# JJKK1313/DiTreeOnlinePlanner

Hardware: AMD Instinct MI355X
Metric: candidate tree-expansions/sec (carmaze, H=32) (higher is better)
Workload: dtype f16x3; 1 GPU; cfgs/carmaze.yaml + fm_policy flow sampler (K=1), batch=1024 candidates per GPU, H=32 (4 chunks x 8 steps), boxes.csv 20x20, 1024-node tree snapshot, seeded random weights; batch_per_gpu=1024, global_batch=1024, edge_length=32, action_horizon=8, pred_horizon=64, flow_steps=1, tree_nodes=1024, parallelism=candidates sharded x1

## Files before the change

### ditreeonlineplanner_amd/csrc/conv_tiles.hip

```cpp
#include <type_traits>

#include "denoise_device.h"

static thread_local bool g_dn_dry_run = false;
void denoise_set_dry_run(bool on) { g_dn_dry_run = on; }
bool denoise_dry_run() { return g_dn_dry_run; }

template <int PREC>
__device__ __forceinline__ void gemm_epilogue(const ConvGemmParams& p, f32x16_t (&acc)[2][4], char* smem, int tm, int tn,
                                              int tid, int lane, int r5, int h, int wm, int wn,
                                              long long out_extra_bytes = 0) {

  constexpr int ET = PREC == 2 ? 1 : 0;
  float satm = 0.0f;
  const int c_l = wn * 128 + 4 * r5;
  const int n0 = tn * 256 + c_l;
  const bool n_ok = n0 < p.N;
  float bias4[4] = {0.f, 0.f, 0.f, 0.f};
  if (p.bias != nullptr && n_ok) {
    f32x4_t t = *(const f32x4_t*)(p.bias + n0);
#pragma unroll
    for (int j = 0; j < 4; ++j) bias4[j] = t[j];
  }
#pragma unroll
// ... 1115 lines not shown
    __builtin_amdgcn_sched_group_barrier(0x008, 16, 0);
    __builtin_amdgcn_sched_barrier(0);
    PSTAMP(3);
    mm16(1, 0, 0);
    if constexpr (ISSUE_A && T != 2) {
      if constexpr (T == 0) { issue_a(v + 1, 0); issue_a(v + 1, 1); issue_a(v + 1, 2); }
      else { issue_a(v + 1, 3); issue_a(v + 1, 4); if constexpr (NP == 6) issue_a(v + 1, 5); }
      __builtin_amdgcn_sched_group_barrier(0x008, 4, 2);
      __builtin_amdgcn_sched_group_barrier(0x020, 1, 2);
      __builtin_amdgcn_sched_group_barrier(0x008, 4, 2);
      __builtin_amdgcn_sched_group_barrier(0x020, 1, 2);
      __builtin_amdgcn_sched_group_barrier(0x008, 4, 2);
      if constexpr (T == 0 || NP == 6) __builtin_amdgcn_sched_group_barrier(0x020, 1, 2);
      __builtin_amdgcn_sched_group_barrier(0x008, 4, 2);
    }
    __builtin_amdgcn_sched_barrier(0);
    PSTAMP(4);
    __builtin_amdgcn_s_setprio(0);
    mm16(0, 1, 1);
    __builtin_amdgcn_sched_barrier(0);
    PSTAMP(5);
    if constexpr (HAS_NEXT) {
      if constexpr (VM == 0) asm volatile("s_waitcnt vmcnt(0) lgkmcnt(0)" ::: "memory");
      else if constexpr (VM == 3) asm volatile("s_waitcnt vmcnt(3) lgkmcnt(0)" ::: "memory");
      else asm volatile("s_waitcnt vmcnt(2) lgkmcnt(0)" ::: "memory");
      __builtin_amdgcn_s_barrier();
      __builtin_amdgcn_s_setprio(3);
      PSTAMP(6);
      constexpr int T1 = (T + 1) % 3;
      rdA(0, v + (T + 1) / 3, T1, 0);
      rdB(0, v + (T + 1) / 3, T1, 1, 0);
    }
    constexpr int T2 = (T + 2) % 3;
    const int v2 = v + (T + 2) / 3;
#pragma unroll
    for (int mb = 0; mb < 4; ++mb)
#pragma unroll
      for (int jj = 0; jj < 4; ++jj) {
        mm(1, 1, 1, mb, (mb & 1) ? 3 - jj : jj);
        const int i = mb * 4 + jj;
        const int d = (i & 1) ? -1 : (i >> 1);
        if constexpr (ISSUE_W) { if (d >= 0 && d < 4) issue_w(v2, T2, d); }
      }
    if constexpr (HAS_NEXT) __builtin_amdgcn_sched_group_barrier(0x100, 8, 1);
    constexpr int NV = ISSUE_W ? 4 : 0;
#pragma unroll
    for (int i = 0; i < 16; ++i) {
      __builtin_amdgcn_sched_group_barrier(0x008, 1, 1);
      if (!(i & 1) && (i >> 1) < NV) __builtin_amdgcn_sched_group_barrier(0x020, 1, 1);
    }
    __builtin_amdgcn_sched_barrier(0);
    PSTAMP(7);
  };
#undef PSTAMP
  using I0 = std::integral_constant<int, 0>;
  using I1 = std::integral_constant<int, 1>;
  using I2 = std::integral_constant<int, 2>;
  using I3 = std::integral_constant<int, 3>;
  using Tt = std::true_type;
  using Ff = std::false_type;

#ifdef HALO16_STAMP
  const unsigned long long xs0 = __builtin_amdgcn_s_memrealtime();
#endif
#pragma unroll
  for (int i = 0; i < NP; ++i) issue_a(v_lo, i);
#pragma unroll
  for (int q = 0; q < 4; ++q) issue_w(v_lo, 0, q);
  asm volatile("s_waitcnt vmcnt(0)" ::: "memory");
  __builtin_amdgcn_s_barrier();
#pragma unroll
  for (int q = 0; q < 4; ++q) issue_w(v_lo, 1, q);
  rdA(0, v_lo, 0, 0);
  rdB(0, v_lo, 0, 1, 0);
#ifdef HALO16_STAMP
  const unsigned long long xs1 = __builtin_amdgcn_s_memrealtime();
#endif

  using IT1 = std::integral_constant<int, NP == 6 ? 3 : 2>;
  for (int v = v_lo; v < nv - 2; ++v) {
    step(I0{}, Tt{}, Tt{}, Tt{}, I3{}, v);
    step(I1{}, Tt{}, Tt{}, Tt{}, IT1{}, v);
    step(I2{}, Tt{}, Tt{}, Tt{}, I0{}, v);
  }
#ifdef X3_PHASE_STAMP
  if (blockIdx.x == 100 && lane == 0 && nv == 64) {
#pragma unroll
    for (int k = 0; k < 24; ++k) g_x3_phase[w][k] = pst[k];
    g_x3_phase[w][24] = (unsigned)nv;
  }
#endif
  {
    const int v = nv - 2;
    step(I0{}, Tt{}, Tt{}, Tt{}, I0{}, v);
    step(I1{}, Tt{}, Tt{}, Tt{}, I0{}, v);
    step(I2{}, Tt{}, Tt{}, Ff{}, I0{}, v);
  }
  {
    const int v = nv - 1;
    step(I0{}, Tt{}, Tt{}, Ff{}, I0{}, v);
    step(I1{}, Tt{}, Ff{}, Ff{}, I0{}, v);
    step(I2{}, Ff{}, Ff{}, Ff{}, I0{}, v);
  }
  __builtin_amdgcn_s_setprio(0);
  __syncthreads();
#ifdef HALO16_STAMP
  const unsigned long long xs2 = __builtin_amdgcn_s_memrealtime();
#endif
  if constexpr (SPLITK) {
    const int ntiles = ntm * ntn;
    float* mine = p.sk_ws + ((size_t)blockIdx.y * ntiles + tile) * 65536;
#pragma unroll
    for (int mb = 0; mb < 4; ++mb)
#pragma unroll
      for (int j = 0; j < 8; ++j) *(f32x4_t*)(mine + ((mb * 8 + j) * 512 + tid) * 4) = acc[mb][j];
    __threadfence();
    __syncthreads();
    int* s_last = (int*)smem;
    if (tid == 0) *s_last = atomicAdd(p.sk_cnt + tile, 1) == p.splitk - 1;
    __syncthreads();
    const bool last = *s_last != 0;
    __syncthreads();
    if (!last) return;
    __threadfence();
#pragma unroll
    for (int mb = 0; mb < 4; ++mb)
#pragma unroll
      for (int j = 0; j < 8; ++j) acc[mb][j] = f32x4_t{0.f, 0.f, 0.f, 0.f};
    for (int sp = 0; sp < p.splitk; ++sp) {
      const float* sl = p.sk_ws + ((size_t)sp * ntiles + tile) * 65536;
#pragma unroll
      for (int mb = 0; mb < 4; ++mb)
#pragma unroll
        for (int j = 0; j < 8; ++j) acc[mb][j] += *(const f32x4_t*)(sl + ((mb * 8 + j) * 512 + tid) * 4);
    }
    if (tid == 0) p.sk_cnt[tile] = 0;
  }
  gemm_epilogue16<ET, true, SHORT>(p, acc, smem, tm, tn, tid, lane, r4, h4, wm, wn);
#ifdef HALO16_STAMP
  __syncthreads();
  if (tid == 0) {
    const unsigned long long xs3 = __builtin_amdgcn_s_memrealtime();
    const unsigned int k = atomicAdd(&g_x3_count, 1u);
    if (k < X3_STAMP_MAX) {
      g_x3_stamp[k][0] = xs0; g_x3_stamp[k][1] = xs1; g_x3_stamp[k][2] = xs2; g_x3_stamp[k][3] = xs3;
      g_x3_stamp[k][4] = ((unsigned long long)nv << 32) | blockIdx.x;
      g_x3_stamp[k][5] = ((unsigned long long)__builtin_amdgcn_s_getreg((31 << 11) | 20) << 32) |
                         (unsigned int)__builtin_amdgcn_s_getreg((31 << 11) | 4);
    }
  }
#endif
}

template <int ET, bool SPLIT>
__global__ void __launch_bounds__(256) conv2d_small_kernel(ConvGemmParams p) {
  extern __shared__ __attribute__((aligned(16))) char smem[];
  constexpr int STAGE = 16384;
  constexpr int CK = SPLIT ? 32 : 64;
  const int tid = threadIdx.x, lane = tid & 63;
  const int w = __builtin_amdgcn_readfirstlane(tid >> 6);
  const int r5 = lane & 31, h = lane >> 5;
  const int wm = w >> 1, wn = w & 1;
  const int ntn = p.N >> 6;
  const int tm = blockIdx.x / ntn, tn = blockIdx.x - tm * ntn;
  const int kpt = p.Cin / CK;
  const long long K = (long long)p.taps * p.Cin;
  int k0 = 0, nk = p.taps * kpt;
  long long out_extra = 0;
  if (p.splitk > 1) {
    const int per = (nk + p.splitk - 1) / p.splitk;
    k0 = blockIdx.y * per;
    nk = min(nk - k0, per);
    out_extra = (long long)blockIdx.y * p.slab_stride;
  }

  const char* a_base[2];
  int ih0[2], iw0[2];
  const char* w_src[2];
  int slot_b[2];
  long long plane_a[2];
#pragma unroll
  for (int q = 0; q < 2; ++q) {
    const int r = (2 * w + q) * 8 + (lane >> 3);
    const int slot = (lane & 7) ^ ((r >> 1) & 7);
    slot_b[q] = SPLIT ? (slot & 3) * 16 : slot * 16;
    plane_a[q] = (SPLIT && (slot & 4)) ? p.a_plane : 0;
    const long long plane_w = (SPLIT && (slot & 4)) ? p.w_plane : 0;
    int m = tm * 64 + r;
    m = m < p.M ? m : p.M - 1;
    const int b = m / p.c2_OHW, rem = m - b * p.c2_OHW;
    const int oh = rem / p.c2_OW, ow = rem - oh * p.c2_OW;
    a_base[q] = (const char*)p.A + (long long)b * p.c2_H * p.c2_W * p.Cin * 2;
    ih0[q] = oh * p.c2_stride - p.c2_pad;
    iw0[q] = ow * p.c2_stride - p.c2_pad;
    w_src[q] = (const char*)p.W + ((long long)(tn * 64 + r) * K) * 2 + slot_b[q] + plane_w;
  }
  auto issue = [&](int kl) {
    const int k = k0 + kl;
    const int tap = k / kpt, kin = k - tap * kpt;
    const int kh = p.c2_kh[tap], kw = p.c2_kw[tap];
    char* st = smem + (kl % 3) * STAGE;
#pragma unroll
    for (int q = 0; q < 2; ++q) {
      const int ih = ih0[q] + kh, iw = iw0[q] + kw;
      const bool ok = ih >= 0 && ih < p.c2_H && iw >= 0 && iw < p.c2_W;
      const char* src = ok ? a_base[q] + ((long long)(ih * p.c2_W + iw) * p.Cin + kin * CK) * 2 + plane_a[q] : (const char*)p.zero;
      __builtin_amdgcn_global_load_lds((const GLOBAL_AS void*)(src + slot_b[q]), (LDS_AS void*)(st + (2 * w + q) * 1024), 16, 0, 0);
    }
#pragma unroll
    for (int q = 0; q < 2; ++q)
      __builtin_amdgcn_global_load_lds((const GLOBAL_AS void*)(w_src[q] + (long long)k * (CK * 2)),
                                       (LDS_AS void*)(st + 8192 + (2 * w + q) * 1024), 16, 0, 0);
  };

  f32x16_t acc;
#pragma unroll
  for (int i = 0; i < 16; ++i) acc[i] = 0.0f;
  const int a_row = wm * 32 + r5, b_row = wn * 32 + r5;
  const int a_off = a_row * 128, b_off = 8192 + b_row * 128;
  const int sa = (a_row >> 1) & 7, sb = (b_row >> 1) & 7;

  issue(0);
  if (nk > 1) issue(1);
  for (int k = 0; k < nk; ++k) {
    if (k + 1 < nk) asm volatile("s_waitcnt vmcnt(4)" ::: "memory");
    else asm volatile("s_waitcnt vmcnt(0)" ::: "memory");
    __builtin_amdgcn_s_barrier();
    if (k + 2 < nk) issue(k + 2);
    const char* st = smem + (k % 3) * STAGE;
    if constexpr (SPLIT) {
      short8_t af[4], bf[4];
#pragma unroll
      for (int ks = 0; ks < 4; ++ks) {
        af[ks] = *(const short8_t*)(st + a_off + ((((ks << 1) | h) ^ sa) << 4));
        bf[ks] = *(const short8_t*)(st + b_off + ((((ks << 1) | h) ^ sb) << 4));
      }
#pragma unroll
      for (int kk = 0; kk < 2; ++kk) acc = mfma32<ET>(af[kk], bf[kk + 2], acc);
#pragma unroll
      for (int kk = 0; kk < 2; ++kk) acc = mfma32<ET>(af[kk], bf[kk], acc);
#pragma unroll
      for (int kk = 0; kk < 2; ++kk) acc = mfma32<ET>(af[kk + 2], bf[kk], acc);
    } else {
#pragma unroll
      for (int ks = 0; ks < 4; ++ks) {
        const short8_t af = *(const short8_t*)(st + a_off + ((((ks << 1) | h) ^ sa) << 4));
        const short8_t bf = *(const short8_t*)(st + b_off + ((((ks << 1) | h) ^ sb) << 4));
        acc = mfma32<ET>(af, bf, acc);
      }
    }
    asm volatile("s_waitcnt lgkmcnt(0)" ::: "memory");
  }

  const int n = tn * 64 + wn * 32 + r5;
  float bias = (p.bias != nullptr && k0 == 0) ? p.bias[n] : 0.0f;
#pragma unroll
  for (int i = 0; i < 16; ++i) {
    const int m = tm * 64 + wm * 32 + (i & 3) + 8 * (i >> 2) + 4 * h;
    if (m < p.M) ((float*)p.Out)[out_extra + (long long)m * p.ldc + p.out_coff + n] = (ET == 1 ? acc[i] * p.w_scale : acc[i]) + bias;
  }
}

template <int ET, bool SPLIT, bool SHORT = false>
__global__ void __launch_bounds__(512, 2) gemm16_kernel(ConvGemmParams p) {
  extern __shared__ __attribute__((aligned(16))) char smem[];
  constexpr int BUF = 32768, W_BASE = 2 * BUF;
  const int tid = threadIdx.x, lane = tid & 63;
  const int w = __builtin_amdgcn_readfirstlane(tid >> 6);
  const int r4 = lane & 15, h4 = lane >> 4;
  const int wm = w >> 1, wn = w & 1;
  const int ntn = p.N >> 8, ntm = p.M >> 8;
  const int tile = xcd_remap_strips(blockIdx.x, ntm, ntn, p.xcd_strips);
  const int tm = tile / ntn, tn = tile - tm * ntn;
  constexpr int KB = SPLIT ? 64 : 128;
  const int nc = SPLIT ? (p.Cin >> 5) : (p.Cin >> 6), nk = p.taps * nc;
  const unsigned a_plane = (unsigned)p.a_plane, w_plane = (unsigned)p.w_plane;
  const long long K = (long long)p.taps * p.Cin;

  long long a_tile0;
  {
    const int m0 = tm * 256;
    const int b0 = m0 / p.L, l0 = m0 - b0 * p.L;
    a_tile0 = (((long long)b0 * p.in_Lp + (long long)l0 * p.in_stride + p.in_off) * p.lda) * 2;
  }
  const __amdgpu_buffer_rsrc_t a_rsrc =
      __builtin_amdgcn_make_buffer_rsrc((void*)((const char*)p.A + a_tile0), 0, 0x7fffffff, 0x00020000);
  const __amdgpu_buffer_rsrc_t w_rsrc =
      __builtin_amdgcn_make_buffer_rsrc((void*)((const char*)p.W + ((long long)tn * 256) * K * 2), 0, 0x7fffffff, 0x00020000);
  unsigned pae, pao, pbe, pbo;
  int aq[4], wq[4];
  {
    const int lr = lane >> 3;
    const int slot0 = (lane & 7) ^ (lr >> 1), slot1 = slot0 ^ 4;
    const int lrb = lr / p.L, lro = lrb * p.in_Lp + (lr - lrb * p.L) * p.in_stride;
    if constexpr (SPLIT) {
      pae = (unsigned)((lro * p.lda + (slot0 & 3) * 8) * 2) + ((slot0 & 4) ? a_plane : 0u);
      pao = (unsigned)((lro * p.lda + (slot1 & 3) * 8) * 2) + ((slot1 & 4) ? a_plane : 0u);
      pbe = (unsigned)(((long long)(8 * lr) * K + (slot0 & 3) * 8) * 2) + ((slot0 & 4) ? w_plane : 0u);
      pbo = (unsigned)(((long long)(8 * lr) * K + (slot1 & 3) * 8) * 2) + ((slot1 & 4) ? w_plane : 0u);
    } else {
      pae = (unsigned)((lro * p.lda + slot0 * 8) * 2);
      pao = (unsigned)((lro * p.lda + slot1 * 8) * 2);
      pbe = (unsigned)(((long long)(8 * lr) * K + slot0 * 8) * 2);
      pbo = (unsigned)(((long long)(8 * lr) * K + slot1 * 8) * 2);
    }
#pragma unroll
    for (int q = 0; q < 4; ++q) {
      const int r0 = (w * 4 + q) * 8;
      const int m = tm * 256 + r0;
      const int b = m / p.L, l = m - b * p.L;
      aq[q] = (int)((((long long)b * p.in_Lp + (long long)l * p.in_stride + p.in_off) * p.lda) * 2 - a_tile0);
      const int cu = (r0 & 128) + 8 * (r0 & 8) + ((r0 >> 4) & 7);
      wq[q] = (int)((long long)cu * K * 2);
    }
  }
  const int tap_bytes = p.lda * 2;
  auto src_off = [&](int k, int& ao, int& wo) {
    const int t = k / nc, c = k - t * nc;
    ao = t * tap_bytes + c * KB;
    wo = k * KB;
  };
  auto issue = [&](int kv) {
    int ao, wo;
    src_off(kv, ao, wo);
    char* ab = smem + (kv & 1) * BUF;
    char* wb = smem + W_BASE + (kv & 1) * BUF;
#pragma unroll
    for (int q = 0; q < 4; ++q)
      __builtin_amdgcn_raw_ptr_buffer_load_lds(a_rsrc, (LDS_AS void*)(ab + (w * 4 + q) * 1024), 16, (q & 1) ? pao : pae,
                                               aq[q] + ao, 0, 0);
#pragma unroll
    for (int q = 0; q < 4; ++q)
      __builtin_amdgcn_raw_ptr_buffer_load_lds(w_rsrc, (LDS_AS void*)(wb + (w * 4 + q) * 1024), 16, (q & 1) ? pbo : pbe,
                                               wq[q] + wo, 0, 0);
  };

  auto issue_wq = [&](int kv, int q) {
    int ao, wo;
    src_off(kv, ao, wo);
    __builtin_amdgcn_raw_ptr_buffer_load_lds(w_rsrc, (LDS_AS void*)(smem + W_BASE + (kv & 1) * BUF + (w * 4 + q) * 1024), 16,
                                             (q & 1) ? pbo : pbe, wq[q] + wo, 0, 0);
  };
  const int a_row = wm * 64 + r4;
  const int swa = (a_row >> 1) & 7;
  const int a_off = a_row * 128, b_off = (wn * 128 + r4) * 128;
  const int swb = (r4 >> 1) & 7;

  f32x4_t acc[4][8];
#pragma unroll
  for (int mb = 0; mb < 4; ++mb)
#pragma unroll
    for (int j = 0; j < 8; ++j) acc[mb][j] = f32x4_t{0.f, 0.f, 0.f, 0.f};
  short8_t af[2][4], bq[2][4];
  auto rdA = [&](int set, int k, int ks) {
    const char* ab = smem + (k & 1) * BUF + a_off + ((((ks << 2) | h4) ^ swa) << 4);
#pragma unroll
    for (int mb = 0; mb < 4; ++mb) af[set][mb] = *(const short8_t*)(ab + mb * 2048);
  };
  auto rdB = [&](int set, int k, int ks, int half) {
    const char* wb = smem + W_BASE + (k & 1) * BUF + b_off + half * 8192 + ((((ks << 2) | h4) ^ swb) << 4);
#pragma unroll
    for (int jj = 0; jj < 4; ++jj) bq[set][jj] = *(const short8_t*)(wb + jj * 2048);
  };
  auto mm = [&](int aset, int bset, int half, int mb, int jj) {
    acc[mb][half * 4 + jj] = mfma16<ET>(af[aset][mb], bq[bset][jj], acc[mb][half * 4 + jj]);
  };
  auto mm16 = [&](int aset, int bset, int half) {
#pragma unroll
    for (int mb = 0; mb < 4; ++mb)
#pragma unroll
      for (int jj = 0; jj < 4; ++jj) mm(aset, bset, half, mb, (mb & 1) ? 3 - jj : jj);
  };
  auto step = [&](auto tNext, auto tIssue, int k) {
    constexpr bool HAS_NEXT = decltype(tNext)::value, ISSUE = decltype(tIssue)::value;
    if constexpr (SPLIT) {
      rdB(1, k, 1, 1);
      mm16(0, 0, 0);
      if constexpr (HAS_NEXT) {
        issue_wq(k + 1, 0); issue_wq(k + 1, 1);
        __builtin_amdgcn_sched_group_barrier(0x100, 4, 0);
        __builtin_amdgcn_sched_group_barrier(0x008, 4, 0);
        __builtin_amdgcn_sched_group_barrier(0x020, 1, 0);
        __builtin_amdgcn_sched_group_barrier(0x008, 4, 0);
        __builtin_amdgcn_sched_group_barrier(0x020, 1, 0);
        __builtin_amdgcn_sched_group_barrier(0x008, 8, 0);
      } else
      {
      __builtin_amdgcn_sched_group_barrier(0x100, 4, 0);
      __builtin_amdgcn_sched_group_barrier(0x008, 16, 0);
      }
      __builtin_amdgcn_sched_barrier(0);
      rdB(0, k, 0, 0);
      rdA(1, k, 1);
      mm16(0, 1, 1);
      if constexpr (HAS_NEXT) {
        issue_wq(k + 1, 2); issue_wq(k + 1, 3);
        __builtin_amdgcn_sched_group_barrier(0x100, 8, 0);
        __builtin_amdgcn_sched_group_barrier(0x008, 4, 0);
        __builtin_amdgcn_sched_group_barrier(0x020, 1, 0);
        __builtin_amdgcn_sched_group_barrier(0x008, 4, 0);
        __builtin_amdgcn_sched_group_barrier(0x020, 1, 0);
        __builtin_amdgcn_sched_group_barrier(0x008, 8, 0);
      } else
      {
      __builtin_amdgcn_sched_group_barrier(0x100, 8, 0);
      __builtin_amdgcn_sched_group_barrier(0x008, 16, 0);
      }
      __builtin_amdgcn_sched_barrier(0);
      rdB(1, k, 0, 1);
      mm16(0, 0, 0);
      __builtin_amdgcn_sched_group_barrier(0x100, 4, 0);
      __builtin_amdgcn_sched_group_barrier(0x008, 16, 0);
      __builtin_amdgcn_sched_barrier(0);
      mm16(1, 0, 0);
      __builtin_amdgcn_sched_barrier(0);
      mm16(0, 1, 1);
      __builtin_amdgcn_sched_barrier(0);
    } else {
      rdB(1, k, 0, 1);
      mm16(0, 0, 0);
      __builtin_amdgcn_sched_group_barrier(0x100, 4, 0);
      __builtin_amdgcn_sched_group_barrier(0x008, 16, 0);
      __builtin_amdgcn_sched_barrier(0);
      rdA(1, k, 1);
      rdB(0, k, 1, 0);
      mm16(0, 1, 1);
      __builtin_amdgcn_sched_group_barrier(0x100, 8, 0);
      __builtin_amdgcn_sched_group_barrier(0x008, 16, 0);
      __builtin_amdgcn_sched_barrier(0);
      rdB(1, k, 1, 1);
      mm16(1, 0, 0);
      __builtin_amdgcn_sched_group_barrier(0x100, 4, 0);
      __builtin_amdgcn_sched_group_barrier(0x008, 16, 0);
      __builtin_amdgcn_sched_barrier(0);
    }
    int ao2 = 0, wo2 = 0;
    if constexpr (ISSUE) src_off(k + 2, ao2, wo2);
    if constexpr (HAS_NEXT) {
      asm volatile("s_waitcnt vmcnt(0) lgkmcnt(0)" ::: "memory");
      __builtin_amdgcn_s_barrier();
      rdA(0, k + 1, 0);
      rdB(0, k + 1, SPLIT ? 1 : 0, 0);
    }
#pragma unroll
    for (int mb = 0; mb < 4; ++mb)
#pragma unroll
      for (int jj = 0; jj < 4; ++jj) {
        mm(1, 1, 1, mb, (mb & 1) ? 3 - jj : jj);
        if constexpr (ISSUE) {
          const int m = mb * 4 + jj, i = (m & 1) ? -1 : (m >> 1);
          if (i >= 0 && i < 4)
            __builtin_amdgcn_raw_ptr_buffer_load_lds(a_rsrc, (LDS_AS void*)(smem + (k & 1) * BUF + (w * 4 + i) * 1024), 16,
                                                     (i & 1) ? pao : pae, aq[i] + ao2, 0, 0);
          else if (!SPLIT && i >= 4 && i < 8)
            __builtin_amdgcn_raw_ptr_buffer_load_lds(w_rsrc, (LDS_AS void*)(smem + W_BASE + (k & 1) * BUF + (w * 4 + i - 4) * 1024),
                                                     16, ((i - 4) & 1) ? pbo : pbe, wq[i - 4] + wo2, 0, 0);
        }
      }
    if constexpr (HAS_NEXT) __builtin_amdgcn_sched_group_barrier(0x100, 8, 1);
#pragma unroll
    for (int i = 0; i < 16; ++i) {
      __builtin_amdgcn_sched_group_barrier(0x008, 1, 1);
      if (ISSUE && !(i & 1) && (!SPLIT || i < 8)) __builtin_amdgcn_sched_group_barrier(0x020, 1, 1);
    }
    __builtin_amdgcn_sched_barrier(0);
  };
  using Tt = std::true_type;
  using Ff = std::false_type;

  issue(0);
  asm volatile("s_waitcnt vmcnt(0)" ::: "memory");
  __builtin_amdgcn_s_barrier();
  if (nk > 1) {
    if constexpr (SPLIT) {
      int ao, wo;
      src_off(1, ao, wo);
#pragma unroll
      for (int q = 0; q < 4; ++q)
        __builtin_amdgcn_raw_ptr_buffer_load_lds(a_rsrc, (LDS_AS void*)(smem + BUF + (w * 4 + q) * 1024), 16, (q & 1) ? pao : pae,
                                                 aq[q] + ao, 0, 0);
    } else {
      issue(1);
    }
  }
  rdA(0, 0, 0);
  rdB(0, 0, SPLIT ? 1 : 0, 0);
  for (int k = 0; k < nk - 2; ++k) step(Tt{}, Tt{}, k);
  if (nk >= 2) step(Tt{}, Ff{}, nk - 2);
  step(Ff{}, Ff{}, nk - 1);
  __syncthreads();
  gemm_epilogue16<ET, SPLIT, SHORT>(p, acc, smem, tm, tn, tid, lane, r4, h4, wm, wn);
}
enum { TILE_HALO, TILE_GEMM16, TILE_C2D_SMALL, TILE_GENERIC };
enum { TV_SPLIT = 1,
       TV_SHORT = 2,
       TV_SPLITK = 4,
       TV_NP6 = 8,
       TV_C2D = 16 };
struct TileVariant {
  void (*kernel)(ConvGemmParams);
  unsigned lds_bytes;
  unsigned block;
  int family, st;
  unsigned flags;
  int kind;
};
static const TileVariant k_tiles[] = {
    {conv3_halo16_kernel<0>, 147456, 512, TILE_HALO, ST_BF16, 0, 0},
    {conv3_halo16_kernel<1>, 147456, 512, TILE_HALO, ST_F16, 0, 0},
    {conv3_halo16x3_kernel<0>, 147456, 512, TILE_HALO, ST_BF16, TV_SPLIT, 0},
    {conv3_halo16x3_kernel<1>, 147456, 512, TILE_HALO, ST_F16, TV_SPLIT, 0},
    {conv3_halo16x3_kernel<0, true>, 147456, 512, TILE_HALO, ST_BF16, TV_SPLIT | TV_SHORT, 0},
    {conv3_halo16x3_kernel<1, true>, 147456, 512, TILE_HALO, ST_F16, TV_SPLIT | TV_SHORT, 0},
    {conv3_halo16x3_kernel<0, false, true>, 147456, 512, TILE_HALO, ST_BF16, TV_SPLIT | TV_SPLITK, 0},
    {conv3_halo16x3_kernel<1, false, true>, 147456, 512, TILE_HALO, ST_F16, TV_SPLIT | TV_SPLITK, 0},
    {conv3_halo16x3_kernel<0, true, true>, 147456, 512, TILE_HALO, ST_BF16, TV_SPLIT | TV_SHORT | TV_SPLITK, 0},
    {conv3_halo16x3_kernel<1, true, true>, 147456, 512, TILE_HALO, ST_F16, TV_SPLIT | TV_SHORT | TV_SPLITK, 0},
    {conv3_halo16x3_kernel<0, true, false, 6>, 163840, 512, TILE_HALO, ST_BF16, TV_SPLIT | TV_SHORT | TV_NP6, 0},
    {conv3_halo16x3_kernel<1, true, false, 6>, 163840, 512, TILE_HALO, ST_F16, TV_SPLIT | TV_SHORT | TV_NP6, 0},
    {gemm16_kernel<0, false>, 131072, 512, TILE_GEMM16, ST_BF16, 0, 1},
    {gemm16_kernel<1, false>, 131072, 512, TILE_GEMM16, ST_F16, 0, 1},
    {gemm16_kernel<0, true>, 131072, 512, TILE_GEMM16, ST_BF16, TV_SPLIT, 1},
    {gemm16_kernel<1, true>, 131072, 512, TILE_GEMM16, ST_F16, TV_SPLIT, 1},
    {gemm16_kernel<0, false, true>, 131072, 512, TILE_GEMM16, ST_BF16, TV_SHORT, 1},
    {gemm16_kernel<1, false, true>, 131072, 512, TILE_GEMM16, ST_F16, TV_SHORT, 1},
    {gemm16_kernel<0, true, true>, 131072, 512, TILE_GEMM16, ST_BF16, TV_SPLIT | TV_SHORT, 1},
    {gemm16_kernel<1, true, true>, 131072, 512, TILE_GEMM16, ST_F16, TV_SPLIT | TV_SHORT, 1},
    {conv2d_small_kernel<0, false>, 3 * 16384, 256, TILE_C2D_SMALL, ST_BF16, TV_C2D, 2},
    {conv2d_small_kernel<1, false>, 3 * 16384, 256, TILE_C2D_SMALL, ST_F16, TV_C2D, 2},
    {conv2d_small_kernel<0, true>, 3 * 16384, 256, TILE_C2D_SMALL, ST_BF16, TV_C2D | TV_SPLIT, 2},
    {conv2d_small_kernel<1, true>, 3 * 16384, 256, TILE_C2D_SMALL, ST_F16, TV_C2D | TV_SPLIT, 2},
    {conv_gemm_kernel<0, false>, 131072, 512, TILE_GENERIC, ST_BF16, 0, 1},
    {conv_gemm_kernel<1, false>, 131072, 512, TILE_GENERIC, ST_F32, 0, 1},
    {conv_gemm_kernel<2, false>, 131072, 512, TILE_GENERIC, ST_F16, 0, 1},
    {conv_gemm_kernel<0, true>, 131072, 512, TILE_GENERIC, ST_BF16, TV_C2D, 2},
    {conv_gemm_kernel<1, true>, 131072, 512, TILE_GENERIC, ST_F32, TV_C2D, 2},
    {conv_gemm_kernel<2, true>, 131072, 512, TILE_GENERIC, ST_F16, TV_C2D, 2},
};
static const TileVariant* find_tile(int family, int st, unsigned flags) {
  for (const TileVariant& v : k_tiles)
    if (v.family == family && v.st == st && v.flags == flags) return &v;
  return nullptr;
}

static const TileVariant* pick_tile(const ConvGemmParams& p, int fmt) {
  const int st = fmt_st(fmt);
  const bool split = fmt_split(fmt);
  const unsigned fsplit = split ? TV_SPLIT : 0;
  const bool tile16 = st != ST_F32 && !p.c2d && (p.M & 255) == 0 && (p.N & 255) == 0 && (p.Cin & 63) == 0;
  const bool l_ok = p.L >= 16 || (p.L == 8 && split) || (p.L == 4 && split && p.splitk <= 1);
  if (tile16 && p.taps == 3 && p.in_stride == 1 && p.in_Lp == p.L + 2 && (256 % p.L) == 0 && l_ok && p.Cin >= 192) {
    if (!split) return find_tile(TILE_HALO, st, 0);
    const unsigned fshort = p.L <= 8 ? TV_SHORT : 0;
    if (p.splitk > 1) return find_tile(TILE_HALO, st, TV_SPLIT | fshort | TV_SPLITK);
    return find_tile(TILE_HALO, st, TV_SPLIT | fshort | (p.L == 4 ? TV_NP6 : 0));
  }
  const bool short_l = p.L == 8 || p.L == 4;
  if (tile16 && (!p.out_f32 || p.mode == MODE_BIAS) && p.taps >= 1 && p.taps <= 3 && ((p.L & 15) == 0 || short_l) && p.M > 0 &&
      (p.mode == MODE_BIAS || (256 % p.L) == 0))
    return find_tile(TILE_GEMM16, st, fsplit | ((p.L & 15) != 0 ? TV_SHORT : 0));
  if (p.c2d && conv2d_small_eligible(fmt) && (p.N & 63) == 0 && (p.Cin & 63) == 0 && p.out_f32 && p.mode == MODE_BIAS)
    return find_tile(TILE_C2D_SMALL, st, TV_C2D | fsplit);
  if (split) return nullptr;
  return find_tile(TILE_GENERIC, st, p.c2d ? TV_C2D : 0);
}
bool conv2d_small_eligible(int fmt) { return fmt_st(fmt) != ST_F32; }
int conv_gemm_kind(const ConvGemmParams& p, int fmt) {
  const TileVariant* v = pick_tile(p, fmt);
  return v != nullptr ? v->kind : (p.c2d ? 2 : 1);
}
bool conv_gemm_supported(const ConvGemmParams& p, int fmt) { return pick_tile(p, fmt) != nullptr; }

static void ensure_lds_attrs() {
  static bool done[64] = {};
  int dev = 0;
  hipGetDevice(&dev);
  if (dev < 0 || dev >= 64 || done[dev]) return;
  done[dev] = true;
  for (const TileVariant& v : k_tiles)
    if (v.lds_bytes > 65536) hipFuncSetAttribute((const void*)v.kernel, hipFuncAttributeMaxDynamicSharedMemorySize, (int)v.lds_bytes);
}

void launch_conv_gemm(const ConvGemmParams& p, int fmt, hipStream_t s) {
  ensure_lds_attrs();
  const TileVariant* v = pick_tile(p, fmt);
  if (v != nullptr && (v->flags & TV_SPLITK) &&
      (p.sk_ws == nullptr || p.sk_cnt == nullptr || ((p.Cin >> 5) % p.splitk) != 0 || (p.Cin >> 5) / p.splitk < 2))
    throw std::runtime_error("conv_gemm: split-K of the halo kernel needs its workspace and splitk | Cin / 32, >= 2 chunks each");
  if ((v == nullptr || v->family == TILE_GENERIC) && p.mode >= MODE_GN_MISH && (p.L & 15) != 0)
    throw std::runtime_error("conv_gemm: a fused GroupNorm epilogue at L = 8 / 4 exists on the gemm16 tile only (whole 256-row tiles)");
  if (v == nullptr) throw std::runtime_error("conv_gemm: a split GEMM of this shape fits no tile (conv_gemm_supported is the contract)");
  dim3 grid(((p.M + 255) >> 8) * ((p.N + 255) >> 8));
  if (v->family == TILE_C2D_SMALL) grid.x = ((p.M + 63) >> 6) * (p.N >> 6);
  if (v->flags & (TV_SPLITK | TV_C2D)) grid.y = p.splitk > 1 ? p.splitk : 1;
  DN_LAUNCH(v->kernel, grid, dim3(v->block), v->lds_bytes, s, p);
}
```

### ditreeonlineplanner_amd/csrc/denoise.h

```cpp
#pragma once
#include <hip/hip_runtime.h>
#include <stdint.h>

enum { MODE_BIAS = 0, MODE_GN_MISH = 1, MODE_GN_MISH_FILM = 2, MODE_GN_MISH_RES = 3 };

enum { ST_BF16 = 0, ST_F32 = 1, ST_F16 = 2 };
static inline int fmt_make(int st, bool split) { return st | (split ? 4 : 0); }
static inline __host__ __device__ int fmt_st(int f) { return f & 3; }
static inline __host__ __device__ bool fmt_split(int f) { return (f & 4) != 0; }
static inline int fmt_es(int f) { return fmt_st(f) == ST_F32 ? 4 : 2; }

struct ConvGemmParams {
  const void* A;
  int lda;
  int in_Lp;
  int in_stride;
  int in_off;
  int taps, Cin;
  const void* W;
  void* Out;
  int ldc;
  int out_Lp, out_stride, out_off;
  int out_coff;
  int L;
  int M, N;
  const float* bias;
  int mode;
  const float* gamma;
  const float* beta;
  int group_ch;
  float eps;
  const float* film;
  int film_ld, film_off;
  const void* Res;
  int ldres, res_Lp, res_off;
  int out_f32;
  int xcd_strips;
  int c2d, c2_H, c2_W, c2_OW, c2_OHW, c2_stride, c2_pad;
  signed char c2_kh[12], c2_kw[12];
  const void* zero;
  long long a_plane, w_plane, out_plane, res_plane;
  float w_scale;
  int splitk;
  long long slab_stride;
  float* sk_ws;
  int* sk_cnt;
  int* sat;
};

void denoise_set_dry_run(bool on);
bool denoise_dry_run();
void launch_conv_gemm(const ConvGemmParams& p, int fmt, hipStream_t s);
bool conv2d_small_eligible(int fmt);
int conv_gemm_kind(const ConvGemmParams& p, int fmt);
bool conv_gemm_supported(const ConvGemmParams& p, int fmt);
void launch_prep_sample(const float* x, void* A0, int B, int P, int D, int fmt, long long plane, hipStream_t s, int* sat = nullptr);
void launch_time_embed(float t, const float* W1, const float* b1, const float* W2, const float* b2, float* out,
                       hipStream_t s);
void launch_prep_cond(const float* temb, const float* map_emb, int E, int E_ld, const float* cond, int G, void* out, int B,
                      int Kpad, int fmt, long long plane, hipStream_t s, int* sat = nullptr);
struct FlowStep {
  int mode;
  float dt;
  float sb, sa, c0, c1, sigma;
  const float* z;
  long long z_row;
  const int* z_idx;
  int z_row0;
};
void launch_final_proj_flow(const void* Y, int C, int Lp, long long plane, const float* W, const float* bias, int D, float* x,
                            FlowStep fs, const double* act_norm , double* actions, int B, int P, int fmt,
                            hipStream_t s);
void launch_gn1d(void* x, int ld, int Lp, int row_off, int coff, int L, int C, const float* gamma, const float* beta, float eps,
                 int mode, const float* film, int film_ld, int film_off, const void* res, int ldres, int res_Lp, int res_off,
                 int B, int fmt, long long x_plane, long long res_plane, hipStream_t s, int* sat = nullptr);
void launch_encoder_stem(const float* lm, int n, const float* W, const float* gamma, const float* beta, void* out, int B, float eps,
                         int fmt, long long plane, hipStream_t s, int* sat = nullptr);
void launch_gn2d(const float* in, int nslab, long long slab_stride, const float* gamma, const float* beta, const void* res,
                 int relu, void* out, int B, int HW, int C, float eps, int fmt, long long res_plane, long long out_plane,
                 hipStream_t s, int* sat = nullptr);
void launch_avgpool2d(const void* in, void* out, int B, int HW, int C, int fmt, long long in_plane, long long out_plane,
                      hipStream_t s);
void launch_unpack_act(const void* in, int ld, int coff, int Lp, int roff, float* out, int B, int L, int C, int fmt,
                       long long plane, hipStream_t s);

enum { ENC_RESNET = 0, ENC_IDENTITY = 1, ENC_MLP = 2, ENC_MAX = 3, ENC_GRID = 4, ENC_CNN = 5 };
struct SmallEncoderParams {
  int kind;
  const float* lm;
  float* out;
  int B, n, E, k;
  const float* w[4];
  const float* b[4];
};
const char* small_encoder_name(int kind);
int small_encoder_width(int kind, int n, int k);
void launch_small_encoder(const SmallEncoderParams& p, hipStream_t s);
```

### ditreeonlineplanner_amd/csrc/denoise_plan.hip

```cpp
#include <algorithm>
#include <cmath>
#include <cstring>
#include <thread>

#include "denoise_state.h"

namespace {

inline uint16_t f2bf_host(float f) {
  uint32_t u;
  std::memcpy(&u, &f, 4);
  if ((u & 0x7fffffffu) > 0x7f800000u) return (uint16_t)((u >> 16) | 0x40);
  u += 0x7fffu + ((u >> 16) & 1u);
  return (uint16_t)(u >> 16);
}
inline float bf2f_host(uint16_t h) {
  uint32_t u = (uint32_t)h << 16;
  float f;
  std::memcpy(&f, &u, 4);
  return f;
}
inline uint16_t f2h_host(float f) { _Float16 h = (_Float16)f; uint16_t u; std::memcpy(&u, &h, 2); return u; }
inline float h2f_host(uint16_t u) { _Float16 h; std::memcpy(&h, &u, 2); return (float)h; }

// ... 342 lines not shown
  std::vector<const float*> wsrc, bsrc;
  std::vector<int> rows, start;
  film_cols = 0;
  for (auto& c : crbs) {
    wsrc.push_back(P_(c + ".cond_encoder.1.weight").data);
    bsrc.push_back(P_(c + ".cond_encoder.1.bias").data);
    rows.push_back((int)P_(c + ".cond_encoder.1.weight").dims[0]);
    start.push_back(film_cols);
    film_cols += rows.back();
  }
  film = (float*)dalloc((size_t)Brows() * film_cols * 4);
  const int cd = cond_dim;
  const Packed wp = pack("film.all", ufmt, film_cols, 1, condK, [=](int n, int, int ci) {
    size_t i = std::upper_bound(start.begin(), start.end(), n) - start.begin() - 1;
    return ci < cd ? wsrc[i][(size_t)(n - start[i]) * cd + ci] : 0.0f;
  });
  std::vector<float> ball(film_cols);
  for (size_t i = 0; i < rows.size(); ++i) std::memcpy(ball.data() + start[i], bsrc[i], (size_t)rows[i] * 4);
  float* bd = upload_f32("film.bias", ball.data(), film_cols);
  ConvGemmParams p = gemm_params(matrix(condA, condK, cond_plane), matrix(film, film_cols), wp, 1, condK, film_cols, 1, 0, 1, 0, 0, bd,
                                 nullptr);
  p.out_f32 = 1;
  const int uf = ufmt;
  film_op = [this, p, uf](int, int Bp, hipStream_t s) { run_rows(p, Bp, fmt_st(uf) != ST_F32, uf, s); };
}

void DenoiserState::build_unet() {
  const int C0 = dims[0], C1 = dims[1], C2 = dims[2];
  const int L0 = P, L1 = P / 2, L2 = P / 4;
  Act a0 = make_act("a0", L0, 64, false);
  const std::string pre = "unet.down_modules.0.0";
  int fc = (int)P_(pre + ".cond_encoder.1.weight").dims[0];
  {
    const float* wd = P_(pre + ".blocks.0.block.0.weight").data;
    const int Dd = D;
    const Packed wp = pack(pre + ".blocks.0.block.0", ufmt, C0, 1, 64, [=](int n, int, int ci) {
      if (ci >= 3 * Dd) return 0.0f;
      const int t = ci / Dd, d = ci - t * Dd;
      return wd[((size_t)n * Dd + d) * 3 + t];
    });
    Act h = make_act("d0b1.h", L0, C0);
    ConvGemmParams p = gemm_params(a0, h, wp, 1, 64, C0, 1, 0, 1, 1, L0, pre + ".blocks.0.block.0");
    set_epilogue(p, MODE_GN_MISH_FILM, pre + ".blocks.0.block.1", 0, nullptr);
    emit_block(p, h);
    const float* wrd = P_(pre + ".residual_conv.weight").data;
    const Packed wrp = pack(pre + ".residual_conv", ufmt, C0, 1, 64, [=](int n, int, int ci) {
      return (ci >= Dd && ci < 2 * Dd) ? wrd[(size_t)n * Dd + (ci - Dd)] : 0.0f;
    });
    Act res = make_act("d0b1.res", L0, C0);
    push_gemm(gemm_params(a0, res, wrp, 1, 64, C0, 1, 0, 1, 1, L0, pre + ".residual_conv"));
    Act o = make_act("d0b1.out", L0, C0);
    add_conv3(pre + ".blocks.1.block.0", h, o, MODE_GN_MISH_RES, pre + ".blocks.1.block.1", 0, &res);
  }
  Act cat1 = make_act("cat1", L1, 2 * C1);
  Act cat0 = make_act("cat0", L2, 2 * C2);
  Act d0o = named["d0b1.out"];
  Act skip0 = make_act("skip0", L0, C0);
  add_crb("unet.down_modules.0.1", d0o, skip0, fc, "d0b2");
  Act d1in = make_act("d1.in", L1, C0);
  add_down("unet.down_modules.0.2.conv", skip0, d1in);
  Act d1o = make_act("d1b1.out", L1, C1);
  add_crb("unet.down_modules.1.0", d1in, d1o, fc, "d1b1");
  Act skip1 = view(cat1, C1, C1);
  named["skip1"] = skip1;
  add_crb("unet.down_modules.1.1", d1o, skip1, fc, "d1b2");
  Act d2in = make_act("d2.in", L2, C1);
  add_down("unet.down_modules.1.2.conv", skip1, d2in);
  Act d2o = make_act("d2b1.out", L2, C2);
  add_crb("unet.down_modules.2.0", d2in, d2o, fc, "d2b1");
  Act skip2 = view(cat0, C2, C2);
  named["skip2"] = skip2;
  add_crb("unet.down_modules.2.1", d2o, skip2, fc, "d2b2");
  Act m1 = make_act("mid1.out", L2, C2);
  add_crb("unet.mid_modules.0", skip2, m1, fc, "mid1");
  Act m2 = view(cat0, 0, C2);
  named["mid2.out"] = m2;
  add_crb("unet.mid_modules.1", m1, m2, fc, "mid2");
  Act u0a = make_act("u0b1.out", L2, C1);
  add_crb("unet.up_modules.0.0", cat0, u0a, fc, "u0b1");
  Act u0b = make_act("u0b2.out", L2, C1);
  add_crb("unet.up_modules.0.1", u0a, u0b, fc, "u0b2");
  Act up0 = view(cat1, 0, C1);
  named["up0.out"] = up0;
  add_up("unet.up_modules.0.2.conv", u0b, up0);
  Act u1a = make_act("u1b1.out", L1, C0);
  add_crb("unet.up_modules.1.0", cat1, u1a, fc, "u1b1");
  Act u1b = make_act("u1b2.out", L1, C0);
  add_crb("unet.up_modules.1.1", u1a, u1b, fc, "u1b2");
  Act fin = make_act("final.in", L0, C0);
  add_up("unet.up_modules.1.2.conv", u1b, fin);
  final_h = make_act("final.h", L0, C0);
  add_conv3("unet.final_conv.0.block.0", fin, final_h, MODE_GN_MISH, "unet.final_conv.0.block.1", 0, nullptr);
  vec("unet.final_conv.1.weight");
  vec("unet.final_conv.1.bias");
  vec("unet.diffusion_step_encoder.1.weight");
  vec("unet.diffusion_step_encoder.1.bias");
  vec("unet.diffusion_step_encoder.3.weight");
  vec("unet.diffusion_step_encoder.3.bias");
}

void DenoiserState::build_encoder_small() {
  SmallEncoderParams q{};
  q.kind = enc_kind; q.n = lm; q.E = E; q.k = enc_k;
  auto transposed = [&](const std::string& name, int out_f, int in_f) {
    const HostParam& w = P_(name);
    if (w.dims.size() != 2 || w.dims[0] != out_f || w.dims[1] != in_f)
      throw std::runtime_error(name + " must be (" + std::to_string(out_f) + ", " + std::to_string(in_f) + ")");
    std::vector<float> t((size_t)out_f * in_f);
    for (int o = 0; o < out_f; ++o)
      for (int i = 0; i < in_f; ++i) t[(size_t)i * out_f + o] = w.data[(size_t)o * in_f + i];
    return upload_f32(name + "#t", t.data(), (int64_t)t.size());
  };
  auto conv_w = [&](const std::string& name, int co, int ci) {
    const HostParam& w = P_(name + ".weight");
    const HostParam& b = P_(name + ".bias");
    if (w.dims.size() != 4 || w.dims[0] != co || w.dims[1] != ci || w.dims[2] != 3 || w.dims[3] != 3 || b.n != co)
      throw std::runtime_error(name + " must be a Conv2d(" + std::to_string(ci) + ", " + std::to_string(co) + ", 3)");
  };
  if (enc_kind == ENC_MLP) {
    const int in_f = lm * lm;
    q.w[0] = transposed("encoder.fc1.weight", 128, in_f);
    q.w[1] = transposed("encoder.fc2.weight", 256, 128);
    q.w[2] = transposed("encoder.fc3.weight", E, 256);
    const int outs[3] = {128, 256, E};
    for (int l = 0; l < 3; ++l) {
      const std::string bn = "encoder.fc" + std::to_string(l + 1) + ".bias";
      if (P_(bn).n != outs[l]) throw std::runtime_error(bn + " must have " + std::to_string(outs[l]) + " elements");
      q.b[l] = vec(bn);
    }
  } else if (enc_kind == ENC_GRID || enc_kind == ENC_CNN) {
    const bool g = enc_kind == ENC_GRID;
    const int nl = g ? 3 : 4;
    const int ci[4] = {1, g ? 3 : 2, g ? 6 : 4, 4}, co[4] = {g ? 3 : 2, g ? 6 : 4, 4, 4};
    for (int l = 0; l < nl; ++l) {
      const std::string nm = "encoder.conv" + std::to_string(l + 1);
      conv_w(nm, co[l], ci[l]);
      q.w[l] = vec(nm + ".weight");
      q.b[l] = vec(nm + ".bias");
    }
  }
  q.out = map_emb;
  enc_ops.push_back([this, q](int B, int, hipStream_t s) {
    prof.note_other();
    SmallEncoderParams r = q;
    r.lm = lm_ptr; r.B = B;
    launch_small_encoder(r, s);
  });
}

void DenoiserState::build_encoder_resnet() {
  const std::string R = "encoder.resnet18.";
  const int pr = efmt;
  const void* zero_row = dalloc(256);
  const size_t gout_per_sample = 9216;
  float* gout = (float*)dalloc((size_t)Bmax * gout_per_sample * 4);
  auto ebuf = [&](const std::string& name, int HW, int C) { return make_act(name, HW, C, false, efmt, HW == 1 ? Brows() : Bmax); };
  auto conv2d = [&](const std::string& wname, const Act& in, int H, int Cout, int k, int stride, int pad, int OH) {
    const HostParam& w = P_(wname + ".weight");
    const float* wd = w.data;
    const int Cw = (int)w.dims[1], Cin = in.C;
    const TapList tl = live_taps(k, stride, pad, H, OH);
    if (Cin % 64 != 0 || tl.n > 12)
      throw std::runtime_error("encoder conv " + wname + " (" + std::to_string(Cin) + " input channels, " + std::to_string(tl.n) +
                               " live taps) fits no implicit-GEMM tile: channels in multiples of 64, at most 12 taps");
    const int K = tl.n * Cin;
    if ((size_t)OH * OH * Cout > gout_per_sample) throw std::runtime_error("encoder scratch region too small for " + wname);
    const Packed wp = pack(wname, efmt, Cout, 1, K, [=](int n, int, int kk) {
      const int c = kk % Cin, t = kk / Cin, kw = tl.kw[t], kh = tl.kh[t];
      return wd[(((size_t)n * Cw + c) * k + kh) * k + kw];
    });
    ConvGemmParams p = gemm_params(in, matrix(gout, Cout), wp, tl.n, Cin, Cout, 1, 0, 1, 0, 0, nullptr, nullptr);
    p.out_f32 = 1;
    p.c2d = 1; p.c2_H = H; p.c2_W = H; p.c2_OW = OH; p.c2_OHW = OH * OH; p.c2_stride = stride; p.c2_pad = pad;
    for (int t = 0; t < tl.n; ++t) { p.c2_kh[t] = tl.kh[t]; p.c2_kw[t] = tl.kw[t]; }
    p.zero = zero_row;
    const int nk_total = tl.n * (Cin / 64);
    const bool small = conv2d_small_eligible(pr);
    const int tiles = small ? ((1024 * OH * OH + 63) / 64) * (Cout / 64) : ((1024 * OH * OH + 255) / 256) * ((Cout + 255) / 256);
    int sk = std::max(1, std::min(std::min(8, nk_total / 2), (small ? 768 : 256) / tiles));
    while (sk > 1 && (size_t)sk * OH * OH * Cout > gout_per_sample) --sk;
    if (sk > 1) {
      const int per = (nk_total + sk - 1) / sk;
      sk = (nk_total + per - 1) / per;
    }
    p.splitk = sk;
    enc_ops.push_back([this, p, pr, OHW = OH * OH](int B, int, hipStream_t s) mutable {
      const int M = B * OHW;
      p.M = M; p.L = M; p.in_Lp = M; p.out_Lp = M;
      p.slab_stride = (long long)M * p.N;
      run_gemm(p, pr, s);
    });
    return sk;
  };
  auto gn = [&](const std::string& gname, int splitk, const Act& out, const Act* res, bool relu) {
    float* ga = vec(gname + ".weight");
    float* be = vec(gname + ".bias");
    const void* rp = res ? res->p : nullptr;
    const int HW = out.L, C = out.C;
    const long long rpl = res ? res->plane : 0;
    {
      const int pp = (C >= 64 && C <= 1024 && (C & (C - 1)) == 0) ? 256 / (C >> 2) : 0;
      if (pp == 0 || (HW + pp - 1) / pp > 7)
        throw std::runtime_error("encoder GroupNorm: unsupported map (" + std::to_string(HW) + " pixels x " + std::to_string(C) + " channels)");
    }
    int* gsat = sat_slot(gname, efmt);
    enc_ops.push_back([=, this](int B, int, hipStream_t s) {
      prof.note_other();
      launch_gn2d(gout, splitk, (long long)B * HW * C, ga, be, rp, relu ? 1 : 0, out.p, B, HW, C, 1e-5f, pr, rpl, out.plane, s, gsat);
    });
  };
  const int H0 = lm;
  auto osz = [](int h, int k, int s, int p) { return (h + 2 * p - k) / s + 1; };
  const int H2 = osz(osz(H0, 7, 2, 3), 3, 2, 1);
  Act pool = ebuf("enc.pool", H2 * H2, 64);
  {
    const HostParam& w = P_(R + "conv1.weight");
    const int Cw = (int)w.dims[1];
    std::vector<float> wf(64 * 49);
    for (int n = 0; n < 64; ++n)
      for (int t = 0; t < 49; ++t) {
        float sacc = 0.f;
        for (int cc = 0; cc < Cw; ++cc) sacc += w.data[((size_t)n * Cw + cc) * 49 + t];
        wf[t * 64 + n] = sacc;
      }
    float* wdev = upload_f32(R + "conv1.weight#folded", wf.data(), 64 * 49);
    float* ga = vec(R + "bn1.weight");
    float* be = vec(R + "bn1.bias");
    int* ssat = sat_slot(R + "conv1", efmt);
    enc_ops.push_back([=, this](int B, int, hipStream_t s) {
      prof.note_other();
      launch_encoder_stem(lm_ptr, H0, wdev, ga, be, pool.p, B, 1e-5f, pr, pool.plane, s, ssat);
    });
  }
  Act cur = pool;
  int Hc = H2;
  const int chans[4] = {64, 128, 256, 512};
  for (int li = 0; li < 4; ++li) {
    for (int bi = 0; bi < 2; ++bi) {
      const std::string pre = R + "layer" + std::to_string(li + 1) + "." + std::to_string(bi);
      const int Cout = chans[li];
      const int stride = (bi == 0 && li > 0) ? 2 : 1;
      const int Ho = osz(Hc, 3, stride, 1);
      const std::string tag = "enc.l" + std::to_string(li + 1) + "." + std::to_string(bi);
      Act t1 = ebuf(tag + ".t", Ho * Ho, Cout);
      gn(pre + ".bn1", conv2d(pre + ".conv1", cur, Hc, Cout, 3, stride, 1, Ho), t1, nullptr, true);
      Act idt = cur;
      if (has(pre + ".downsample.0.weight")) {
        Act ds = ebuf(tag + ".ds", Ho * Ho, Cout);
        gn(pre + ".downsample.1", conv2d(pre + ".downsample.0", cur, Hc, Cout, 1, stride, 0, Ho), ds, nullptr, false);
        idt = ds;
      }
      Act o = ebuf(tag + ".out", Ho * Ho, Cout);
      gn(pre + ".bn2", conv2d(pre + ".conv2", t1, Ho, Cout, 3, 1, 1, Ho), o, &idt, true);
      cur = o;
      Hc = Ho;
    }
  }
  Act pooled = ebuf("enc.avg", 1, cur.C);
  enc_ops.push_back([=, this](int B, int, hipStream_t s) {
    prof.note_other();
    launch_avgpool2d(cur.p, pooled.p, B, cur.L, cur.C, pr, cur.plane, pooled.plane, s);
  });
  {
    const HostParam& w = P_(R + "fc.weight");
    const float* wd = w.data;
    const int Kf = (int)w.dims[1], Nf = (int)w.dims[0];
    const Packed wp = pack(R + "fc", efmt, Nf, 1, Kf, [=](int n, int, int ci) { return wd[(size_t)n * Kf + ci]; });
    const bool esplit = fmt_split(efmt);
    float* bd;
    if (esplit) {
      std::vector<float> bpad(E_ld, 0.0f);
      std::memcpy(bpad.data(), P_(R + "fc.bias").data, (size_t)Nf * 4);
      bd = upload_f32(R + "fc.bias#padded", bpad.data(), E_ld);
    } else {
      bd = vec(R + "fc.bias");
    }
    ConvGemmParams p = gemm_params(matrix(pooled.p, Kf, pooled.plane), matrix(map_emb, E_ld), wp, 1, Kf, esplit ? E_ld : Nf, 1, 0, 1, 0,
                                   0, bd, nullptr);
    p.out_f32 = 1;
    enc_ops.push_back([this, p, pr, esplit](int B, int, hipStream_t s) { run_rows(p, B, esplit, pr, s); });
  }
}

void DenoiserState::validate_plan() {
  float* lm_dev = (float*)dalloc((size_t)bgran * lm * lm * 4);
  lm_ptr = lm_dev;
  denoise_set_dry_run(true);
  try {
    for (auto& op : enc_ops) op(bgran, bgran, nullptr);
    film_op(bgran, bgran, nullptr);
    for (auto& op : unet_ops) op(bgran, bgran, nullptr);
  } catch (...) {
    denoise_set_dry_run(false);
    lm_ptr = nullptr;
    throw;
  }
  denoise_set_dry_run(false);
  lm_ptr = nullptr;
}
```

Before: 19210 candidate expansions/s.

## Add position-major conv tiles that skip padded taps in small encoder convs

Adds a position-major variant of the small implicit-GEMM conv kernel. Each tile covers 64 samples at a single output position, so it can compute which taps fall in the padding and skip their K-chunks entirely instead of loading zero rows and running MFMAs on them. Positions are stable-sorted by live-tap count so the heaviest tiles are scheduled first. The cost is more templated variants, per-block tap-mask logic, a strided output scatter, and a limit of 32 output positions, which makes it apply only to the deepest encoder layers.

```diff
diff --git a/ditreeonlineplanner_amd/csrc/conv_tiles.hip b/ditreeonlineplanner_amd/csrc/conv_tiles.hip
--- a/ditreeonlineplanner_amd/csrc/conv_tiles.hip
+++ b/ditreeonlineplanner_amd/csrc/conv_tiles.hip
@@ -1291,7 +1291,7 @@
 #endif
 }
 
-template <int ET, bool SPLIT>
+template <int ET, bool SPLIT, bool POS>
 __global__ void __launch_bounds__(256) conv2d_small_kernel(ConvGemmParams p) {
   extern __shared__ __attribute__((aligned(16))) char smem[];
   constexpr int STAGE = 16384;
@@ -1312,6 +1312,22 @@
     nk = min(nk - k0, per);
     out_extra = (long long)blockIdx.y * p.slab_stride;
   }
+  const int nB = POS ? p.M / p.c2_OHW : 0, ntb = (nB + 63) >> 6;
+  const int tpos = POS ? tm / ntb : 0, b0 = POS ? (tm - tpos * ntb) * 64 : 0;
+  const int pos = POS ? p.c2_order[tpos] : 0;
+  const int poh = pos / p.c2_OW, pih0 = poh * p.c2_stride - p.c2_pad, piw0 = (pos - poh * p.c2_OW) * p.c2_stride - p.c2_pad;
+  unsigned live = 0;
+  int nl = nk;
+  if constexpr (POS) {
+    nl = 0;
+    for (int t = 0; t < p.taps; ++t) {
+      const int ih = pih0 + p.c2_kh[t], iw = piw0 + p.c2_kw[t];
+      if (ih >= 0 && ih < p.c2_H && iw >= 0 && iw < p.c2_W) {
+        live |= 1u << t;
+        nl += max(0, min(k0 + nk, (t + 1) * kpt) - max(k0, t * kpt));
+      }
+    }
+  }
 
   const char* a_base[2];
   int ih0[2], iw0[2];
@@ -1325,24 +1341,36 @@
     slot_b[q] = SPLIT ? (slot & 3) * 16 : slot * 16;
     plane_a[q] = (SPLIT && (slot & 4)) ? p.a_plane : 0;
     const long long plane_w = (SPLIT && (slot & 4)) ? p.w_plane : 0;
-    int m = tm * 64 + r;
-    m = m < p.M ? m : p.M - 1;
-    const int b = m / p.c2_OHW, rem = m - b * p.c2_OHW;
-    const int oh = rem / p.c2_OW, ow = rem - oh * p.c2_OW;
+    int b;
+    if constexpr (POS) {
+      b = min(b0 + r, nB - 1);
+      ih0[q] = pih0;
+      iw0[q] = piw0;
+    } else {
+      int m = tm * 64 + r;
+      m = m < p.M ? m : p.M - 1;
+      b = m / p.c2_OHW;
+      const int rem = m - b * p.c2_OHW;
+      const int oh = rem / p.c2_OW, ow = rem - oh * p.c2_OW;
+      ih0[q] = oh * p.c2_stride - p.c2_pad;
+      iw0[q] = ow * p.c2_stride - p.c2_pad;
+    }
     a_base[q] = (const char*)p.A + (long long)b * p.c2_H * p.c2_W * p.Cin * 2;
-    ih0[q] = oh * p.c2_stride - p.c2_pad;
-    iw0[q] = ow * p.c2_stride - p.c2_pad;
     w_src[q] = (const char*)p.W + ((long long)(tn * 64 + r) * K) * 2 + slot_b[q] + plane_w;
   }
+  int kn = k0;
   auto issue = [&](int kl) {
-    const int k = k0 + kl;
+    if constexpr (POS) {
+      for (int t = kn / kpt; !((live >> t) & 1u);) kn = ++t * kpt;
+    }
+    const int k = kn++;
     const int tap = k / kpt, kin = k - tap * kpt;
     const int kh = p.c2_kh[tap], kw = p.c2_kw[tap];
     char* st = smem + (kl % 3) * STAGE;
 #pragma unroll
     for (int q = 0; q < 2; ++q) {
       const int ih = ih0[q] + kh, iw = iw0[q] + kw;
-      const bool ok = ih >= 0 && ih < p.c2_H && iw >= 0 && iw < p.c2_W;
+      const bool ok = POS || (ih >= 0 && ih < p.c2_H && iw >= 0 && iw < p.c2_W);
       const char* src = ok ? a_base[q] + ((long long)(ih * p.c2_W + iw) * p.Cin + kin * CK) * 2 + plane_a[q] : (const char*)p.zero;
       __builtin_amdgcn_global_load_lds((const GLOBAL_AS void*)(src + slot_b[q]), (LDS_AS void*)(st + (2 * w + q) * 1024), 16, 0, 0);
     }
@@ -1359,13 +1387,13 @@
   const int a_off = a_row * 128, b_off = 8192 + b_row * 128;
   const int sa = (a_row >> 1) & 7, sb = (b_row >> 1) & 7;
 
-  issue(0);
-  if (nk > 1) issue(1);
-  for (int k = 0; k < nk; ++k) {
-    if (k + 1 < nk) asm volatile("s_waitcnt vmcnt(4)" ::: "memory");
+  if (nl > 0) issue(0);
+  if (nl > 1) issue(1);
+  for (int k = 0; k < nl; ++k) {
+    if (k + 1 < nl) asm volatile("s_waitcnt vmcnt(4)" ::: "memory");
     else asm volatile("s_waitcnt vmcnt(0)" ::: "memory");
     __builtin_amdgcn_s_barrier();
-    if (k + 2 < nk) issue(k + 2);
+    if (k + 2 < nl) issue(k + 2);
     const char* st = smem + (k % 3) * STAGE;
     if constexpr (SPLIT) {
       short8_t af[4], bf[4];
@@ -1395,7 +1423,8 @@
   float bias = (p.bias != nullptr && k0 == 0) ? p.bias[n] : 0.0f;
 #pragma unroll
   for (int i = 0; i < 16; ++i) {
-    const int m = tm * 64 + wm * 32 + (i & 3) + 8 * (i >> 2) + 4 * h;
+    const int r = wm * 32 + (i & 3) + 8 * (i >> 2) + 4 * h;
+    const int m = POS ? (b0 + r) * p.c2_OHW + pos : tm * 64 + r;
     if (m < p.M) ((float*)p.Out)[out_extra + (long long)m * p.ldc + p.out_coff + n] = (ET == 1 ? acc[i] * p.w_scale : acc[i]) + bias;
   }
 }
@@ -1635,7 +1664,8 @@
        TV_SHORT = 2,
        TV_SPLITK = 4,
        TV_NP6 = 8,
-       TV_C2D = 16 };
+       TV_C2D = 16,
+       TV_POS = 32 };
 struct TileVariant {
   void (*kernel)(ConvGemmParams);
   unsigned lds_bytes;
@@ -1665,10 +1695,14 @@
     {gemm16_kernel<1, false, true>, 131072, 512, TILE_GEMM16, ST_F16, TV_SHORT, 1},
     {gemm16_kernel<0, true, true>, 131072, 512, TILE_GEMM16, ST_BF16, TV_SPLIT | TV_SHORT, 1},
     {gemm16_kernel<1, true, true>, 131072, 512, TILE_GEMM16, ST_F16, TV_SPLIT | TV_SHORT, 1},
-    {conv2d_small_kernel<0, false>, 3 * 16384, 256, TILE_C2D_SMALL, ST_BF16, TV_C2D, 2},
-    {conv2d_small_kernel<1, false>, 3 * 16384, 256, TILE_C2D_SMALL, ST_F16, TV_C2D, 2},
-    {conv2d_small_kernel<0, true>, 3 * 16384, 256, TILE_C2D_SMALL, ST_BF16, TV_C2D | TV_SPLIT, 2},
-    {conv2d_small_kernel<1, true>, 3 * 16384, 256, TILE_C2D_SMALL, ST_F16, TV_C2D | TV_SPLIT, 2},
+    {conv2d_small_kernel<0, false, false>, 3 * 16384, 256, TILE_C2D_SMALL, ST_BF16, TV_C2D, 2},
+    {conv2d_small_kernel<1, false, false>, 3 * 16384, 256, TILE_C2D_SMALL, ST_F16, TV_C2D, 2},
+    {conv2d_small_kernel<0, true, false>, 3 * 16384, 256, TILE_C2D_SMALL, ST_BF16, TV_C2D | TV_SPLIT, 2},
+    {conv2d_small_kernel<1, true, false>, 3 * 16384, 256, TILE_C2D_SMALL, ST_F16, TV_C2D | TV_SPLIT, 2},
+    {conv2d_small_kernel<0, false, true>, 3 * 16384, 256, TILE_C2D_SMALL, ST_BF16, TV_C2D | TV_POS, 2},
+    {conv2d_small_kernel<1, false, true>, 3 * 16384, 256, TILE_C2D_SMALL, ST_F16, TV_C2D | TV_POS, 2},
+    {conv2d_small_kernel<0, true, true>, 3 * 16384, 256, TILE_C2D_SMALL, ST_BF16, TV_C2D | TV_SPLIT | TV_POS, 2},
+    {conv2d_small_kernel<1, true, true>, 3 * 16384, 256, TILE_C2D_SMALL, ST_F16, TV_C2D | TV_SPLIT | TV_POS, 2},
     {conv_gemm_kernel<0, false>, 131072, 512, TILE_GENERIC, ST_BF16, 0, 1},
     {conv_gemm_kernel<1, false>, 131072, 512, TILE_GENERIC, ST_F32, 0, 1},
     {conv_gemm_kernel<2, false>, 131072, 512, TILE_GENERIC, ST_F16, 0, 1},
@@ -1699,7 +1733,7 @@
       (p.mode == MODE_BIAS || (256 % p.L) == 0))
     return find_tile(TILE_GEMM16, st, fsplit | ((p.L & 15) != 0 ? TV_SHORT : 0));
   if (p.c2d && conv2d_small_eligible(fmt) && (p.N & 63) == 0 && (p.Cin & 63) == 0 && p.out_f32 && p.mode == MODE_BIAS)
-    return find_tile(TILE_C2D_SMALL, st, TV_C2D | fsplit);
+    return find_tile(TILE_C2D_SMALL, st, TV_C2D | fsplit | (p.c2_pos ? TV_POS : 0));
   if (split) return nullptr;
   return find_tile(TILE_GENERIC, st, p.c2d ? TV_C2D : 0);
 }
@@ -1731,6 +1765,10 @@
   if (v == nullptr) throw std::runtime_error("conv_gemm: a split GEMM of this shape fits no tile (conv_gemm_supported is the contract)");
   dim3 grid(((p.M + 255) >> 8) * ((p.N + 255) >> 8));
   if (v->family == TILE_C2D_SMALL) grid.x = ((p.M + 63) >> 6) * (p.N >> 6);
+  if (v->flags & TV_POS) {
+    if (p.c2_OHW > C2_MAX_POS || p.M % p.c2_OHW != 0) throw std::runtime_error("conv_gemm: position-major tiles need whole samples and a listed position order");
+    grid.x = p.c2_OHW * ((p.M / p.c2_OHW + 63) >> 6) * (p.N >> 6);
+  }
   if (v->flags & (TV_SPLITK | TV_C2D)) grid.y = p.splitk > 1 ? p.splitk : 1;
   DN_LAUNCH(v->kernel, grid, dim3(v->block), v->lds_bytes, s, p);
 }
diff --git a/ditreeonlineplanner_amd/csrc/denoise.h b/ditreeonlineplanner_amd/csrc/denoise.h
--- a/ditreeonlineplanner_amd/csrc/denoise.h
+++ b/ditreeonlineplanner_amd/csrc/denoise.h
@@ -9,6 +9,8 @@
 static inline __host__ __device__ int fmt_st(int f) { return f & 3; }
 static inline __host__ __device__ bool fmt_split(int f) { return (f & 4) != 0; }
 static inline int fmt_es(int f) { return fmt_st(f) == ST_F32 ? 4 : 2; }
+
+enum { C2_MAX_POS = 32 };
 
 struct ConvGemmParams {
   const void* A;
@@ -39,6 +41,8 @@
   int c2d, c2_H, c2_W, c2_OW, c2_OHW, c2_stride, c2_pad;
   signed char c2_kh[12], c2_kw[12];
   const void* zero;
+  int c2_pos;
+  unsigned char c2_order[C2_MAX_POS];
   long long a_plane, w_plane, out_plane, res_plane;
   float w_scale;
   int splitk;
diff --git a/ditreeonlineplanner_amd/csrc/denoise_plan.hip b/ditreeonlineplanner_amd/csrc/denoise_plan.hip
--- a/ditreeonlineplanner_amd/csrc/denoise_plan.hip
+++ b/ditreeonlineplanner_amd/csrc/denoise_plan.hip
@@ -518,6 +518,8 @@
   const std::string R = "encoder.resnet18.";
   const int pr = efmt;
   const void* zero_row = dalloc(256);
+  const char* pos_env = getenv("DITREE_ENC_POSITION_TILES");
+  const bool pos_tiles = pos_env == nullptr || atoi(pos_env) != 0;
   const size_t gout_per_sample = 9216;
   float* gout = (float*)dalloc((size_t)Bmax * gout_per_sample * 4);
   auto ebuf = [&](const std::string& name, int HW, int C) { return make_act(name, HW, C, false, efmt, HW == 1 ? Brows() : Bmax); };
@@ -540,6 +542,19 @@
     p.c2d = 1; p.c2_H = H; p.c2_W = H; p.c2_OW = OH; p.c2_OHW = OH * OH; p.c2_stride = stride; p.c2_pad = pad;
     for (int t = 0; t < tl.n; ++t) { p.c2_kh[t] = tl.kh[t]; p.c2_kw[t] = tl.kw[t]; }
     p.zero = zero_row;
+    if (pos_tiles && conv2d_small_eligible(pr) && OH * OH <= C2_MAX_POS) {
+      auto taps_at = [&](int pos) {
+        int n = 0;
+        for (int t = 0; t < tl.n; ++t) {
+          const int ih = (pos / OH) * stride - pad + tl.kh[t], iw = (pos % OH) * stride - pad + tl.kw[t];
+          n += ih >= 0 && ih < H && iw >= 0 && iw < H;
+        }
+        return n;
+      };
+      p.c2_pos = 1;
+      for (int i = 0; i < OH * OH; ++i) p.c2_order[i] = (unsigned char)i;
+      std::stable_sort(p.c2_order, p.c2_order + OH * OH, [&](int a, int b) { return taps_at(a) > taps_at(b); });
+    }
     const int nk_total = tl.n * (Cin / 64);
     const bool small = conv2d_small_eligible(pr);
     const int tiles = small ? ((1024 * OH * OH + 63) / 64) * (Cout / 64) : ((1024 * OH * OH + 255) / 256) * ((Cout + 255) / 256);
```

New measurement: 19270 candidate expansions/s, median of 6. No clear change (+0.3%).
